# fal-ai-community/video-diffusion-speedrun

Measured on AMD Instinct MI355X. Metric: train-step samples/sec (video latents), higher is better.
Workload: dtype bf16; 1 GPU; C3b DiT-XL/2 bf16, latents [16,16,64,64] pt=2 -> 8192+16 tokens, ctx [512,4096]; per_gpu_batch=12, global_batch=12, parallelism=single, launch=eager, deterministic=False

## Files before the change

### video_diffusion_speedrun_amd/csrc/config.h

```cpp
#pragma once
#include <cstddef>

namespace vdscfg {
enum Knob {
  GEMM_TILE,
  GEMM_NARROW,
  GEMM_GROUP_M,
  GEMM_GROUP_M_TN,
  GEMM_TN_JOINT,
  GEMM_MID_TN,
  GEMM_MID_FACTOR,
  ATTN_MFMA16,
  ATTN_DELTA_FOLD,
  ATTN_TAIL_LAST,
  ATTN_FWD_WIDE,
  ATTN_WIDE_STORES,
  ATTN_QSPLIT,
  CROSS_DKV16,
  ATTN8_DQ_WAVES,
  EW_MIN_ROWS,
  EW_WGS,
  RMSNORM_Q4,
  ROPE_TOK,
  ROPE_TILE,
  ADALN_MFMA,
  COMM_ALLPAIRS,
  DETERMINISTIC,
  N_KNOBS
};
extern double g_val[N_KNOBS];
inline double get(Knob k) { return g_val[k]; }
inline int geti(Knob k) { return (int)g_val[k]; }
const char* rccl_path();
}

namespace vdsdet {
inline bool on() { return vdscfg::g_val[vdscfg::DETERMINISTIC] != 0; }
float* workspace(size_t floats, const char* who);
size_t workspace_bytes();
}
```

### video_diffusion_speedrun_amd/csrc/config.hip

```cpp
#include "config.h"
#include "common.h"
#include "../../include/vds.h"
#include <cmath>
#include <cstdint>
#include <cstdlib>
#include <cstring>

namespace vdscfg {
namespace {
struct Def { const char* name; const char* env; double def; };
const Def kDefs[N_KNOBS] = {
    {"gemm_tile", "VDS_GEMM_TILE", 0},
    {"gemm_narrow", "VDS_GEMM_NARROW", 1},
    {"gemm_group_m", "VDS_GEMM_GROUP_M", 4},
    {"gemm_group_m_tn", "VDS_GEMM_GROUP_M_TN", 0},
    {"gemm_tn_joint", "VDS_GEMM_TN_JOINT", 1},
    {"gemm_mid_tn", "VDS_GEMM_MID_TN", 0.75},
    {"gemm_mid_factor", "VDS_GEMM_MID_FACTOR", 1.3},
    {"attn_mfma16", "VDS_ATTN_MFMA16", 7},
    {"attn_delta_fold", "VDS_ATTN_DELTA_FOLD", 1},
    {"attn_tail_last", "VDS_ATTN_TAIL_LAST", 1},
    {"attn_fwd_wide", "VDS_ATTN_FWD_WIDE", 2},
    {"attn_wide_stores", "VDS_ATTN_WIDE_STORES", 1},
    {"attn_qsplit", "VDS_ATTN_QSPLIT", 0},
    {"cross_dkv16", "VDS_CROSS_DKV16", 1},
    {"attn8_dq_waves", "VDS_ATTN8_DQ_WAVES", 4},
    {"ew_min_rows", "VDS_EW_MIN_ROWS", 8},
    {"ew_wgs", "VDS_EW_WGS", 768},
    {"rmsnorm_q4", "VDS_RMSNORM_Q4", 1},
    {"rope_tok", "VDS_ROPE_TOK", 1},
    {"rope_tile", "VDS_ROPE_TILE", 4},
    {"adaln_mfma", "VDS_ADALN_MFMA", 1},
    {"comm_allpairs", nullptr, 0},
    {"deterministic", nullptr, 0},
};
const char* g_rccl_path = nullptr;
const char* env(const char* name) { return name ? getenv(name) : nullptr; }
struct Init {
  Init() {
    for (int i = 0; i < N_KNOBS; ++i) {
      const char* e = env(kDefs[i].env);
      g_val[i] = (e && *e) ? atof(e) : kDefs[i].def;
    }
    const char* s = env("VDS_COMM_SCHEDULE");
    if (s && strcmp(s, "allpairs") == 0) g_val[COMM_ALLPAIRS] = 1;
    g_rccl_path = env("VDS_RCCL_PATH");
  }
};
}
double g_val[N_KNOBS];
static Init g_init;
const char* rccl_path() { return g_rccl_path; }
}

namespace vdsdet {
static float* g_ws = nullptr;
static size_t g_ws_bytes = 0;
float* workspace(size_t floats, const char* who) {
  if (g_ws && floats * 4 <= g_ws_bytes) return g_ws;
  vdserr::set("%s: deterministic mode needs %zu bytes of workspace, vds_set_deterministic was given %zu", who, floats * 4,
              g_ws_bytes);
  return nullptr;
}
size_t workspace_bytes() { return g_ws ? g_ws_bytes : 0; }
}

extern "C" int vds_set_deterministic(int32_t on, void* workspace, size_t workspace_bytes) {
  const int prev = vdscfg::geti(vdscfg::DETERMINISTIC);
  if (on != 0 && on != 1) return VDS_ERR_ARG;
  if (on && (!workspace || ((uintptr_t)workspace & 15) || workspace_bytes < 4096)) return VDS_ERR_ARG;
  vdscfg::g_val[vdscfg::DETERMINISTIC] = on;
  vdsdet::g_ws = on ? (float*)workspace : nullptr;
  vdsdet::g_ws_bytes = on ? workspace_bytes : 0;
  return prev;
}

extern "C" int vds_knob_set(const char* name, double value) {
  if (!name) return VDS_ERR_ARG;
  for (int i = 0; i < vdscfg::N_KNOBS; ++i)
    if (strcmp(name, vdscfg::kDefs[i].name) == 0) {
      if (i == vdscfg::DETERMINISTIC) return VDS_ERR_ARG;
      vdscfg::g_val[i] = value;
      return VDS_OK;
    }
  return VDS_ERR_ARG;
}

extern "C" double vds_knob_get(const char* name) {
  if (name)
    for (int i = 0; i < vdscfg::N_KNOBS; ++i)
      if (strcmp(name, vdscfg::kDefs[i].name) == 0) return vdscfg::g_val[i];
  return NAN;
}
```

### video_diffusion_speedrun_amd/csrc/gemm.hip

```cpp
#include "common.h"
#include "prof.h"
#include "config.h"
#include "../../include/vds.h"
#include <cmath>
#include <cstdint>
#include <cstring>
#include <mutex>
#include <type_traits>

#ifndef VDS_GEMM_AUX_NT
#define VDS_GEMM_AUX_NT 1
#endif
namespace {

constexpr int BM = 128, BN = 128, BK = 64;
constexpr int TILE_BYTES = 16384;
constexpr int EPI_LD = 68;
constexpr int LDS_BYTES = 4 * 64 * EPI_LD * 4;
constexpr int GROUP_M = 8;

struct GemmP {
  int M, N, K;
  const bf16_t* A; long lda;
  const bf16_t* B; long ldb;
  void* C; long ldc;
  void* C2; long ldc2;
  const bf16_t* bias;
  const bf16_t* aux; long ldaux;
  const float* gate; long ldgate;
  int rows_per_batch;
  int row_base;
  int split_k;
  int atomic;
  long slab_stride;
  unsigned a_bytes, b_bytes;
  int tiles_m, tiles_n;
  int group_m;
  int joint_xcd;
  int narrow;
  const float* sa; const float* sb;
  double prof_k;
  unsigned char* e_q; long e_ldq; unsigned char* e_qt; long e_ldqt;
  const float* e_amax_in; float* e_amax_out; float* e_dq_out; int e_fmt; float* e_colsum;
};

__device__ __forceinline__ int swz_kc(int row, int chunk) { return chunk ^ ((row >> 1) & 7); }
__device__ __forceinline__ int swz_km(int krow) { return (krow & 3) | (((krow >> 3) & 1) << 2); }

template <bool KMAJOR>
__device__ __forceinline__ void stage_tile(srd_t rsrc, char* lds_tile, const unsigned voff[4],
                                           unsigned koff, int wave, int lane, int krem) {
  const unsigned base = lds_addr_of(lds_tile) + wave * 4096;
#pragma unroll
  for (int j = 0; j < 4; ++j) {
    unsigned off = voff[j] + koff;
    if constexpr (!KMAJOR) {
      if (krem < BK) {
        const int row = (wave * 4 + j) * 8 + (lane >> 3);
        if (swz_kc(row, lane & 7) * 8 >= krem) off = 0xfffffff0u;
      }
    }
    lds_dma16(rsrc, base + j * 1024, off);
  }
}

template <bool KMAJOR>
__device__ __forceinline__ void stage_offsets(unsigned voff[4], int wave, int lane, long ld, int origin) {
#pragma unroll
  for (int j = 0; j < 4; ++j) {
    int q = wave * 4 + j;
    if constexpr (!KMAJOR) {
      int row = q * 8 + (lane >> 3);
      int chunk = swz_kc(row, lane & 7);
      voff[j] = (unsigned)(((long)(origin + row) * ld + chunk * 8) * 2);
    } else {
      int krow = q * 4 + (lane >> 4);
      int pc = lane & 15;
      int chunk = (((pc >> 1) ^ swz_km(krow)) << 1) | (pc & 1);
      voff[j] = (unsigned)(((long)krow * ld + origin + chunk * 8) * 2);
    }
  }
}

__device__ __forceinline__ bf16x8 frag_kc(const char* tile, int row0, int ks, int lane) {
  int row = row0 + (lane & 15);
  int chunk = swz_kc(row, ks * 4 + (lane >> 4));
  return *reinterpret_cast<const bf16x8*>(tile + row * 128 + chunk * 16);
}
__device__ __forceinline__ bf16x8 frag_km(const char* tile, int col0, int ks, int lane) {
  int g = lane >> 4, i = lane & 15;
  int krow = ks * 32 + 8 * g + (i >> 2);
  int seg = (col0 >> 4) ^ swz_km(krow);
  const char* p = tile + krow * 256 + seg * 32 + (i & 3) * 8;
  s16x4 lo = __builtin_amdgcn_ds_read_tr16_b64_v4i16((__attribute__((address_space(3))) s16x4*)LDS_PTR(p));
  s16x4 hi = __builtin_amdgcn_ds_read_tr16_b64_v4i16((__attribute__((address_space(3))) s16x4*)LDS_PTR(p + 4 * 256));
  s16x8 r = {lo[0], lo[1], lo[2], lo[3], hi[0], hi[1], hi[2], hi[3]};
  return __builtin_bit_cast(bf16x8, r);
}

typedef __attribute__((ext_vector_type(8))) int i32x8;
__device__ __forceinline__ i32x8 frag_kc8(const char* tile, int row0, int lane) {
  const int row = row0 + (lane & 15);
  const int c0 = swz_kc(row, 2 * (lane >> 4));
  const i32x4 lo = *reinterpret_cast<const i32x4*>(tile + row * 128 + c0 * 16);
  const i32x4 hi = *reinterpret_cast<const i32x4*>(tile + row * 128 + (c0 ^ 1) * 16);
  return i32x8{lo[0], lo[1], lo[2], lo[3], hi[0], hi[1], hi[2], hi[3]};
}

constexpr int LUT_N = 4096, LUT_BYTES = LUT_N * 4, LUT_E0 = 114;
__device__ float g_gelu_lut[2][LUT_N];
typedef __attribute__((ext_vector_type(2))) float f32x2;
typedef __attribute__((ext_vector_type(2))) unsigned short u16x2;

__device__ __forceinline__ f32x2 lut_pair(const char* lut, unsigned w) {
  u16x2 m = __builtin_bit_cast(u16x2, w & 0x7fff7fffu);
  m = __builtin_elementwise_sub_sat(m, u16x2{LUT_E0 << 7, LUT_E0 << 7});
  m = __builtin_elementwise_min(m, u16x2{2047, 2047});
  m = m << u16x2{2, 2};
  const unsigned off = __builtin_bit_cast(unsigned, m) | ((w >> 2) & 0x20002000u);
  f32x2 t;
  t[0] = *reinterpret_cast<const float*>(lut + (off & 0xffffu));
  t[1] = *reinterpret_cast<const float*>(lut + (off >> 16));
  return t;
}
__device__ __forceinline__ f32x2 bf2_to_f2(unsigned w) { return f32x2{bflo(w), bfhi(w)}; }
__device__ __forceinline__ unsigned f2_to_bf2(f32x2 v) { return pack_bf2(v[0], v[1]); }

bool ensure_gelu_lut() {
  static std::mutex mu;
  static bool done[64] = {};
  int dev = 0;
  if (hipGetDevice(&dev) != hipSuccess || dev < 0 || dev >= 64) return false;
  std::lock_guard<std::mutex> lk(mu);
  if (done[dev]) return true;
  static float host[2][LUT_N];
  for (int i = 0; i < LUT_N; ++i) {
    const unsigned bits = (unsigned)(((i & 2047) + (LUT_E0 << 7)) | ((i >> 11) << 15)) << 16;
    float xf;
    memcpy(&xf, &bits, 4);
    const double x = xf;
    const double cdf = 0.5 * erfc(-x * 0.70710678118654752440);
    const double pdf = 0.39894228040143267794 * exp(-0.5 * x * x);
    host[0][i] = (float)cdf;
    host[1][i] = (float)(cdf + x * pdf);
  }
  if (hipMemcpyToSymbol(HIP_SYMBOL(g_gelu_lut), host, sizeof(host)) != hipSuccess) return false;
  done[dev] = true;
  return true;
}

__device__ __forceinline__ unsigned cvt4_fp8(int fmt, float a, float b, float c, float d) {
  int w = 0;
  if (fmt == 0) {
    w = __builtin_amdgcn_cvt_pk_fp8_f32(a, b, w, false);
    w = __builtin_amdgcn_cvt_pk_fp8_f32(c, d, w, true);
  } else {
    w = __builtin_amdgcn_cvt_pk_bf8_f32(a, b, w, false);
    w = __builtin_amdgcn_cvt_pk_bf8_f32(c, d, w, true);
  }
  return (unsigned)w;
}

template <int EPI, int WC = 64, int NIT = 8>
__device__ __forceinline__ void epilogue_prefetch(const GemmP& p, int row0, int col0, int lane, u32x4 (&auxr)[NIT]) {
  if constexpr (EPI == VDS_EPI_GATE_RES || EPI == VDS_EPI_DGELU) {
    const int c8 = lane & 7, rin = lane >> 3;
    const int gcol = col0 + c8 * 8;
    const bool cok = gcol < p.N && (WC == 64 || c8 * 8 < WC);
#pragma unroll
    for (int it = 0; it < NIT; ++it) {
      const long grow = row0 + it * 8 + rin;
#if VDS_GEMM_AUX_NT
      auxr[it] = (grow < p.M && cok) ? __builtin_nontemporal_load(reinterpret_cast<const u32x4*>(p.aux + grow * p.ldaux + gcol))
                                     : u32x4{0u, 0u, 0u, 0u};
#else
      auxr[it] = (grow < p.M && cok) ? *reinterpret_cast<const u32x4*>(p.aux + grow * p.ldaux + gcol)
                                     : u32x4{0u, 0u, 0u, 0u};
#endif
    }
  }
}

template <int EPI, bool EMIT = false, bool LUT = false, int WC = 64, int NIT = 8>
__device__ __forceinline__ void epilogue_64x64(const GemmP& p, float* stg, int row0, int col0, int lane,
                                               float (&cs)[8], u32x2 (&ew)[NIT], const u32x4 (&auxr)[NIT],
                                               const char* lut = nullptr) {
  if constexpr (EPI == VDS_EPI_F32) {
    if (p.atomic) {
      const int acol = col0 + lane;
      if (acol < p.N && lane < WC) {
        float* cbase = reinterpret_cast<float*>(p.C) + (long)row0 * p.ldc + acol;
        const int rmax = min(8 * NIT, p.M - row0);
// ... 599 lines not shown
        for (int j = 0; j < 2; ++j) acc[qa * 4 + i][j] = mma(fa[i][ks], fb0[j][ks], acc[qa * 4 + i][j]);
  };
  auto k_tile = [&](int T, auto PAR) {
    constexpr int par = decltype(PAR)::value;
    const char* buf = ring + par * BUF;
    read_a4(buf + SLOT_A0, fa);
    read_b2(buf + SLOT_B0, fb0);
    issue(T + 1, 3, par ^ 1);
    VDS_WAIT_LGKM0();
    VDS_WAIT_VM(6);
    __builtin_amdgcn_s_barrier();
    __builtin_amdgcn_s_setprio(1);
    quad(0);
    __builtin_amdgcn_s_setprio(0);
    __builtin_amdgcn_s_barrier();
    read_a4(buf + SLOT_A1, fa);
    issue(T + 2, 0, par);
    issue(T + 2, 1, par);
    VDS_WAIT_LGKM0();
    VDS_WAIT_VM(6);
    __builtin_amdgcn_s_barrier();
    __builtin_amdgcn_s_setprio(1);
    quad(1);
    __builtin_amdgcn_s_setprio(0);
    __builtin_amdgcn_s_barrier();
  };
  for (int T = kt_begin; T < kt_end; T += 2) {
    k_tile(T, std::integral_constant<int, 0>{});
    if (T + 1 < kt_end) k_tile(T + 1, std::integral_constant<int, 1>{});
  }
  }
  constexpr int NIT = 8;
  constexpr int NSTEP = 16 / NIT;
  constexpr int RSTEP = 8 * NIT;
  u32x4 auxr2[NSTEP][NIT];
#pragma unroll
  for (int st = 0; st < NSTEP; ++st)
    epilogue_prefetch<EPI, G::WCOLS, NIT>(p, m0 + wr * 128 + st * RSTEP, n0 + wc * G::WCOLS, lane, auxr2[st]);
  if (wr == 0) __builtin_amdgcn_s_barrier();
  const bool aux_all = (EPI == VDS_EPI_GATE_RES || EPI == VDS_EPI_DGELU) && m0 + wr * 128 + 128 <= p.M &&
                       n0 + (wc + 1) * G::WCOLS <= p.N;
  if (aux_all) VDS_WAIT_VM(16);
  else VDS_WAIT_VM(0);
  __builtin_amdgcn_s_barrier();

  constexpr int STG_BASE = 0, STG_WAVE = RSTEP * EPI_LD;
  float* stg = reinterpret_cast<float*>(ring + STG_BASE) + wave * STG_WAVE;
  float dq = 1.0f;
  if constexpr (FMT != 0) dq = (p.sa ? *p.sa : 1.0f) * (p.sb ? *p.sb : 1.0f);
  constexpr bool EMIT = (FMT != 0 && (EPI == VDS_EPI_BIAS_GELU || EPI == VDS_EPI_DGELU)) || (FMT == 0 && EPI == VDS_EPI_DGELU);
  float cs[8];
  u32x2 ew[NSTEP][NIT];
#pragma unroll
  for (int e = 0; e < 8; ++e) cs[e] = 0.f;
  [[maybe_unused]] float e_scale = 1.0f, e_max = 0.f;
  if constexpr (EMIT) {
    const float fmax = p.e_fmt == 0 ? 448.0f : 57344.0f;
    const float ain = ((p.e_q || p.e_qt) && p.e_amax_in) ? *p.e_amax_in : 0.f;
    e_scale = ain > 0.f ? fmax / ain : 1.0f;
    if ((p.e_q || p.e_qt) && p.e_dq_out && m0 == 0 && n0 == 0 && tid == 0) *p.e_dq_out = ain > 0.f ? ain / fmax : 1.0f;
  }
  const char* lut = smem;
#pragma unroll
  for (int qa = 0; qa < NSTEP; ++qa) {
    const u32x4 (&auxr)[NIT] = auxr2[qa];
    const int row0 = m0 + wr * 128 + qa * RSTEP, col0 = n0 + wc * WCOLS;
#pragma unroll
    for (int i = 0; i < RSTEP / 16; ++i)
#pragma unroll
      for (int j = 0; j < NJ; ++j) {
        f32x4 v = acc[qa * (RSTEP / 16) + i][j];
        if constexpr (FMT != 0) v *= dq;
        *reinterpret_cast<f32x4*>(stg + (i * 16 + (lane & 15)) * EPI_LD + j * 16 + 4 * (lane >> 4)) = v;
      }
    VDS_WAIT_LGKM0();
    __builtin_amdgcn_wave_barrier();
    bool full = row0 + RSTEP <= p.M && col0 + WCOLS <= p.N;
    if constexpr (EPI == VDS_EPI_GATE_RES) full = full && ((row0 + p.row_base) % p.rows_per_batch) + RSTEP <= p.rows_per_batch;
    if constexpr (EPI == VDS_EPI_F32) full = false;
    bool done = false;
    if (full) done = epilogue_full_dispatch<EPI, EMIT, WCOLS, NIT>(p, stg, lut, row0, col0, lane, cs, ew[qa], auxr, e_scale, e_max);
    if (!done) epilogue_64x64<EPI, EMIT, USE_LUT, WCOLS, NIT>(p, stg, row0, col0, lane, cs, ew[qa], auxr, lut);
    __builtin_amdgcn_wave_barrier();
  }
  if constexpr (EMIT) {
    if ((p.e_q || p.e_qt) && p.e_amax_out) {
#pragma unroll
      for (int o = 32; o > 0; o >>= 1) e_max = fmaxf(e_max, __shfl_xor(e_max, o));
      unsigned* a = reinterpret_cast<unsigned*>(p.e_amax_out);
      if (lane == 0 && __float_as_uint(e_max) > __atomic_load_n(a, __ATOMIC_RELAXED)) atomicMax(a, __float_as_uint(e_max));
    }
  }
  if constexpr (EMIT) {
    if (p.e_qt) {
      constexpr int TLD = 72;
      unsigned char* bt = reinterpret_cast<unsigned char*>(stg);
      const int c8 = lane & 7, rin = lane >> 3;
#pragma unroll
      for (int qa = 0; qa < NSTEP; ++qa)
#pragma unroll
        for (int it = 0; it < NIT; ++it) *reinterpret_cast<u32x2*>(bt + (qa * RSTEP + it * 8 + rin) * TLD + c8 * 8) = ew[qa][it];
      VDS_WAIT_LGKM0();
      __builtin_amdgcn_wave_barrier();
      const int mq = lane & 31;
      const long m = m0 + wr * 128 + 4 * mq;
#pragma unroll
      for (int it = 0; it < 8; ++it) {
        const int kq = (lane >> 5) + 2 * it;
        unsigned r[4];
#pragma unroll
        for (int i = 0; i < 4; ++i) r[i] = *reinterpret_cast<const unsigned*>(bt + (4 * mq + i) * TLD + 4 * kq);
        const unsigned t0 = __builtin_amdgcn_perm(r[1], r[0], 0x05010400u), t1 = __builtin_amdgcn_perm(r[1], r[0], 0x07030602u);
        const unsigned t2 = __builtin_amdgcn_perm(r[3], r[2], 0x05010400u), t3 = __builtin_amdgcn_perm(r[3], r[2], 0x07030602u);
        const unsigned c[4] = {__builtin_amdgcn_perm(t2, t0, 0x05040100u), __builtin_amdgcn_perm(t2, t0, 0x07060302u),
                               __builtin_amdgcn_perm(t3, t1, 0x05040100u), __builtin_amdgcn_perm(t3, t1, 0x07060302u)};
#pragma unroll
        for (int j = 0; j < 4; ++j) {
          const int col = n0 + wc * WCOLS + 4 * kq + j;
          if (col >= p.N || m >= p.M || 4 * kq + j >= WCOLS) continue;
          unsigned char* dst = p.e_qt + (long)col * p.e_ldqt + m;
          if (m + 4 <= p.M) *reinterpret_cast<unsigned*>(dst) = c[j];
          else
            for (int i = 0; i < (int)(p.M - m); ++i) dst[i] = (unsigned char)(c[j] >> (8 * i));
        }
      }
      VDS_WAIT_LGKM0();
      __builtin_amdgcn_wave_barrier();
    }
    if (p.e_colsum) {
#pragma unroll
      for (int e = 0; e < 8; ++e) {
        cs[e] += __shfl_xor(cs[e], 8);
        cs[e] += __shfl_xor(cs[e], 16);
        cs[e] += __shfl_xor(cs[e], 32);
      }
      if (wr == 1 && lane < 8)
#pragma unroll
        for (int e = 0; e < 8; ++e) stg[lane * 8 + e] = cs[e];
      __syncthreads();
      if (wr == 0 && lane < WCOLS / 8) {
        const float* other = reinterpret_cast<const float*>(ring + STG_BASE) + (wave + 4) * STG_WAVE;
        const int gcol = n0 + wc * WCOLS + lane * 8;
#pragma unroll
        for (int e = 0; e < 8; ++e)
          if (gcol + e < p.N) atomicAdd(p.e_colsum + gcol + e, cs[e] + other[lane * 8 + e]);
      }
    }
  }
}

template <int LAYOUT, int EPI, int FMT = 0>
__global__ __launch_bounds__(512, 2) void gemm_kernel(GemmP p) {
  extern __shared__ __attribute__((aligned(16))) char smem[];
  const int nwg = p.tiles_m * p.tiles_n;
  int pid = blockIdx.x;
  {
    int q = nwg >> 3, r = nwg & 7, xcd = pid & 7, idx = pid >> 3;
    pid = (xcd < r ? xcd * (q + 1) : r * (q + 1) + (xcd - r) * q) + idx;
  }
  const int group = p.group_m * p.tiles_n;
  const int first_m = (pid / group) * p.group_m;
  const int gsz = min(p.tiles_m - first_m, p.group_m);
  const int tile_m = first_m + (pid % group) % gsz;
  const int tile_n = (pid % group) / gsz;
  const int m0 = tile_m * BM, n0 = tile_n * 256;

  const int kt_total = (p.K + BK - 1) / BK;
  int kt_begin = 0, kt_end = kt_total;
  if (p.split_k > 1) {
    int per = (kt_total + p.split_k - 1) / p.split_k;
    kt_begin = blockIdx.y * per;
    kt_end = min(kt_total, kt_begin + per);
    if (kt_begin >= kt_end) return;
  }
  if (p.narrow && tile_n == p.tiles_n - 1) {
    gemm_tile<LAYOUT, EPI, FMT, 128>(p, smem, m0, n0, kt_begin, kt_end);
    return;
  }
  gemm_tile<LAYOUT, EPI, FMT, 256>(p, smem, m0, n0, kt_begin, kt_end);
}

template <int LAYOUT, int EPI, int FMT = 0>
int launch(const GemmP& p, hipStream_t s) {
  constexpr bool USE_LUT = EPI == VDS_EPI_BIAS_GELU || EPI == VDS_EPI_DGELU;
  constexpr int LDS_TOTAL = LDS_BYTES + (USE_LUT ? LUT_BYTES : 0);
  static bool attr_set = false;
  if (!attr_set) {
    (void)hipFuncSetAttribute(reinterpret_cast<const void*>(&gemm_kernel<LAYOUT, EPI, FMT>),
                              hipFuncAttributeMaxDynamicSharedMemorySize, LDS_TOTAL);
    attr_set = true;
  }
  if constexpr (USE_LUT) {
    if (!ensure_gelu_lut()) return VDS_ERR_LAUNCH;
  }
  dim3 grid(p.tiles_m * p.tiles_n, p.split_k > 1 ? p.split_k : 1, 1);
  const double k = FMT != 0 ? p.prof_k : (double)p.K;
  vdsprof::Scope ps(FMT != 0 ? VDS_PROF_GEMM_FP8 : LAYOUT == VDS_NT ? VDS_PROF_GEMM_NT : LAYOUT == VDS_NN ? VDS_PROF_GEMM_NN
                                                                                                       : VDS_PROF_GEMM_TN,
                    s, 2.0 * p.M * p.N * k, (FMT != 0 ? 1.0 : 2.0) * ((double)p.M * k + (double)p.N * k) + 2.0 * (double)p.M * p.N);
  hipLaunchKernelGGL((gemm_kernel<LAYOUT, EPI, FMT>), grid, dim3(512), LDS_TOTAL, s, p);
  return hipGetLastError() == hipSuccess ? VDS_OK : VDS_ERR_LAUNCH;
}

}

namespace mid {
constexpr int BM = 256, BN = 128, BK = 32;
constexpr int A_BYTES = 16384, B_BYTES = 8192, STAGE = A_BYTES + B_BYTES;
constexpr int LDS_BYTES = 3 * STAGE;
static_assert(LDS_BYTES >= 4 * 64 * EPI_LD * 4, "epilogue staging must fit in the stage ring");

__device__ __forceinline__ int swz32(int row) {
  const int h = (row >> 2) & 3;
  return (((h >> 1) ^ h) & 1) << 1 | (h >> 1);
}

template <bool KMAJOR, int ROWS>
__device__ __forceinline__ void offsets(unsigned (&voff)[ROWS / 64], int (&kchunk)[ROWS / 64], int wave, int lane,
                                        long ld, int origin) {
  constexpr int NP = ROWS / 64;
#pragma unroll
  for (int j = 0; j < NP; ++j) {
    const int q = wave * NP + j;
    if constexpr (!KMAJOR) {
      const int row = q * 16 + (lane >> 2);
      const int chunk = (lane & 3) ^ swz32(row);
      kchunk[j] = chunk * 8;
      voff[j] = (unsigned)(((long)(origin + row) * ld + chunk * 8) * 2);
    } else {
      const int t = q >> 3, krow = (q & 7) * 4 + (lane >> 4);
      const int pc = lane & 15;
      const int chunk = (((pc >> 1) ^ swz_km(krow)) << 1) | (pc & 1);
      kchunk[j] = krow;
      voff[j] = (unsigned)(((long)krow * ld + origin + t * 128 + chunk * 8) * 2);
    }
  }
}

template <bool KMAJOR, int NP>
__device__ __forceinline__ void issue(srd_t rsrc, char* slot, const unsigned (&voff)[NP], const int (&kchunk)[NP],
                                      unsigned koff, int krem, int wave) {
  const unsigned base = lds_addr_of(slot) + wave * NP * 1024;
#pragma unroll
  for (int j = 0; j < NP; ++j) {
    unsigned off = voff[j] + koff;
    if (kchunk[j] >= krem) off = 0xfffffff0u;
    lds_dma16(rsrc, base + j * 1024, off);
  }
}

__device__ __forceinline__ bf16x8 frag_kc32(const char* tile, int row0, int lane) {
  const int row = row0 + (lane & 15);
  const int pc = (lane >> 4) ^ swz32(row);
  return *reinterpret_cast<const bf16x8*>(tile + row * 64 + pc * 16);
}

template <int LAYOUT, int EPI>
__global__ __launch_bounds__(256, 2) void gemm_kernel(GemmP p) {
  extern __shared__ __attribute__((aligned(16))) char smem[];
  constexpr bool A_KM = (LAYOUT == VDS_TN);
  constexpr bool B_KM = (LAYOUT != VDS_NT);
  const int tid = threadIdx.x, lane = tid & 63;
  const int wave = __builtin_amdgcn_readfirstlane(tid >> 6);
  const int wm = wave >> 1, wn = wave & 1;

  const int nwg = p.tiles_m * p.tiles_n;
  int pid = blockIdx.x, split = blockIdx.y;
  if (p.split_k > 1 && p.joint_xcd) {
    const int total = nwg * p.split_k;
    int L = blockIdx.y * nwg + blockIdx.x;
    const int q = total >> 3, r = total & 7, xcd = L & 7, idx = L >> 3;
    L = (xcd < r ? xcd * (q + 1) : r * (q + 1) + (xcd - r) * q) + idx;
    split = L / nwg;
    pid = L - split * nwg;
  } else {
    int q = nwg >> 3, r = nwg & 7, xcd = pid & 7, idx = pid >> 3;
    pid = (xcd < r ? xcd * (q + 1) : r * (q + 1) + (xcd - r) * q) + idx;
  }
  const int group = p.group_m * p.tiles_n;
  const int first_m = (pid / group) * p.group_m;
  const int gsz = min(p.tiles_m - first_m, p.group_m);
  const int tile_m = first_m + (pid % group) % gsz;
  const int tile_n = (pid % group) / gsz;
  const int m0 = tile_m * BM, n0 = tile_n * BN;

  const int kt_total = (p.K + BK - 1) / BK;
  int kt_begin = 0, kt_end = kt_total;
  if (p.split_k > 1) {
    int per = (kt_total + p.split_k - 1) / p.split_k;
    kt_begin = split * per;
    kt_end = min(kt_total, kt_begin + per);
    if (kt_begin >= kt_end) return;
  }

  const srd_t ra = make_srd(p.A, p.a_bytes);
  const srd_t rb = make_srd(p.B, p.b_bytes);
  unsigned va[4], vb[2];
  int ca[4], cb[2];
  offsets<A_KM, 256>(va, ca, wave, lane, p.lda, m0);
  offsets<B_KM, 128>(vb, cb, wave, lane, p.ldb, n0);
  const unsigned a_step = A_KM ? (unsigned)(BK * p.lda * 2) : BK * 2;
  const unsigned b_step = B_KM ? (unsigned)(BK * p.ldb * 2) : BK * 2;

  auto stage_in = [&](int T, int slot) {
    const int krem = (T < kt_end) ? p.K - T * BK : 0;
    char* st = smem + slot * STAGE;
    issue<A_KM, 4>(ra, st, va, ca, (unsigned)T * a_step, krem, wave);
    issue<B_KM, 2>(rb, st + A_BYTES, vb, cb, (unsigned)T * b_step, krem, wave);
  };

  f32x4 acc[8][4];
#pragma unroll
  for (int i = 0; i < 8; ++i)
#pragma unroll
    for (int j = 0; j < 4; ++j) acc[i][j] = f32x4{0.f, 0.f, 0.f, 0.f};

  stage_in(kt_begin, 0);
  stage_in(kt_begin + 1, 1);
  VDS_WAIT_VM(6);
  __builtin_amdgcn_s_barrier();

  auto k_step = [&](int T, auto SLOT) {
    constexpr int slot = decltype(SLOT)::value;
    stage_in(T + 2, (slot + 2) % 3);
    const char* ta = smem + slot * STAGE;
    const char* tb = ta + A_BYTES;
    bf16x8 fa[8], fb[4];
#pragma unroll
    for (int i = 0; i < 8; ++i) {
      if constexpr (A_KM) fa[i] = frag_km(ta + wm * B_BYTES, i * 16, 0, lane);
      else fa[i] = frag_kc32(ta, wm * 128 + i * 16, lane);
    }
#pragma unroll
    for (int j = 0; j < 4; ++j) {
      if constexpr (B_KM) fb[j] = frag_km(tb, wn * 64 + j * 16, 0, lane);
      else fb[j] = frag_kc32(tb, wn * 64 + j * 16, lane);
    }
    __builtin_amdgcn_s_setprio(1);
#pragma unroll
    for (int i = 0; i < 8; ++i)
#pragma unroll
      for (int j = 0; j < 4; ++j) acc[i][j] = __builtin_amdgcn_mfma_f32_16x16x32_bf16(fa[i], fb[j], acc[i][j], 0, 0, 0);
    __builtin_amdgcn_s_setprio(0);
    VDS_WAIT_VM(6);
    __builtin_amdgcn_s_barrier();
  };
  for (int T = kt_begin; T < kt_end; T += 3) {
    k_step(T, std::integral_constant<int, 0>{});
    if (T + 1 < kt_end) k_step(T + 1, std::integral_constant<int, 1>{});
    if (T + 2 < kt_end) k_step(T + 2, std::integral_constant<int, 2>{});
  }
  VDS_WAIT_VM(0);
  __builtin_amdgcn_s_barrier();

  float* stg = reinterpret_cast<float*>(smem) + wave * 64 * EPI_LD;
  float cs_unused[8];
  u32x2 ew_unused[8];
#pragma unroll
  for (int qa = 0; qa < 2; ++qa) {
    u32x4 auxr[8];
    epilogue_prefetch<EPI>(p, m0 + wm * 128 + qa * 64, n0 + wn * 64, lane, auxr);
#pragma unroll
    for (int i = 0; i < 4; ++i)
#pragma unroll
      for (int j = 0; j < 4; ++j)
#pragma unroll
        for (int r = 0; r < 4; ++r)
          stg[(i * 16 + 4 * (lane >> 4) + r) * EPI_LD + j * 16 + (lane & 15)] = acc[qa * 4 + i][j][r];
    VDS_WAIT_LGKM0();
    __builtin_amdgcn_wave_barrier();
    epilogue_64x64<EPI>(p, stg, m0 + wm * 128 + qa * 64, n0 + wn * 64, lane, cs_unused, ew_unused, auxr);
    __builtin_amdgcn_wave_barrier();
  }
}

template <int LAYOUT, int EPI>
int launch(const GemmP& p, hipStream_t s) {
  static bool attr_set = false;
  if (!attr_set) {
    (void)hipFuncSetAttribute(reinterpret_cast<const void*>(&gemm_kernel<LAYOUT, EPI>),
                              hipFuncAttributeMaxDynamicSharedMemorySize, LDS_BYTES);
    attr_set = true;
  }
  dim3 grid(p.tiles_m * p.tiles_n, p.split_k > 1 ? p.split_k : 1, 1);
  vdsprof::Scope ps(LAYOUT == VDS_NT ? VDS_PROF_GEMM_NT : LAYOUT == VDS_NN ? VDS_PROF_GEMM_NN : VDS_PROF_GEMM_TN, s,
                    2.0 * p.M * p.N * p.K, 2.0 * ((double)p.M * p.K + (double)p.N * p.K + (double)p.M * p.N));
  hipLaunchKernelGGL((gemm_kernel<LAYOUT, EPI>), grid, dim3(256), LDS_BYTES, s, p);
  return hipGetLastError() == hipSuccess ? VDS_OK : VDS_ERR_LAUNCH;
}
}

thread_local char g_err[256] = "";

template <int LAYOUT, int EPI>
int launch(const GemmP& p, hipStream_t s) {
  static bool attr_set = false;
  if (!attr_set) {
    (void)hipFuncSetAttribute(reinterpret_cast<const void*>(&gemm_kernel<LAYOUT, EPI>),
                              hipFuncAttributeMaxDynamicSharedMemorySize, LDS_BYTES);
    attr_set = true;
  }
  dim3 grid(p.tiles_m * p.tiles_n, p.split_k > 1 ? p.split_k : 1, 1);
  vdsprof::Scope ps(LAYOUT == VDS_NT ? VDS_PROF_GEMM_NT : LAYOUT == VDS_NN ? VDS_PROF_GEMM_NN : VDS_PROF_GEMM_TN, s,
                    2.0 * p.M * p.N * p.K, 2.0 * ((double)p.M * p.K + (double)p.N * p.K + (double)p.M * p.N));
  hipLaunchKernelGGL((gemm_kernel<LAYOUT, EPI>), grid, dim3(256), LDS_BYTES, s, p);
  return hipGetLastError() == hipSuccess ? VDS_OK : VDS_ERR_LAUNCH;
}


__global__ __launch_bounds__(256) void splitk_reduce_kernel(const float* ws, int n_slabs, long slab_stride, float* C, long ldc,
                                                            int M, int N) {
  const long i4 = (long)blockIdx.x * 256 + threadIdx.x;
  const int n4 = N >> 2;
  if (i4 >= (long)M * n4) return;
  const long row = i4 / n4;
  const int col = (int)(i4 % n4) * 4;
  float* c = C + row * ldc + col;
  f32x4 v = *reinterpret_cast<const f32x4*>(c);
  const float* w = ws + row * N + col;
  for (int sidx = 0; sidx < n_slabs; ++sidx) v += *reinterpret_cast<const f32x4*>(w + (long)sidx * slab_stride);
  *reinterpret_cast<f32x4*>(c) = v;
}

inline int force_tile() { return vdscfg::geti(vdscfg::GEMM_TILE); }

inline int narrow_last_column(long N) {
  if (!vdscfg::geti(vdscfg::GEMM_NARROW)) return 0;
  const long rem = N % 256;
  return rem > 0 && rem <= 128;
}

template <typename F>
int launch_split_det(GemmP& p, float* C, long ldc, hipStream_t s, int bk, F launch_fn) {
  const int kt_total = cdiv(p.K, bk);
  int split = p.split_k;
  const size_t slab = (size_t)p.M * p.N * 4;
  while (split > 1 && (size_t)split * slab > vdsdet::workspace_bytes()) --split;
  if (split <= 1) {
    p.split_k = 1;
    return launch_fn(p);
  }
  const int per = cdiv(kt_total, split);
  const int n_eff = cdiv(kt_total, per);
  float* ws = vdsdet::workspace((size_t)split * p.M * p.N, "vds_gemm (split-K)");
  if (!ws) return VDS_ERR_ARG;
  p.split_k = split;
  p.atomic = 0;
  p.joint_xcd = 0;
  p.C = ws;
  p.ldc = p.N;
  p.slab_stride = (long)p.M * p.N;
  const int rc = launch_fn(p);
  if (rc != VDS_OK) return rc;
  const long n4 = (long)p.M * (p.N >> 2);
  hipLaunchKernelGGL(splitk_reduce_kernel, dim3((unsigned)((n4 + 255) / 256)), dim3(256), 0, s, (const float*)ws, n_eff,
                     p.slab_stride, C, ldc, p.M, p.N);
  return hipGetLastError() == hipSuccess ? VDS_OK : VDS_ERR_LAUNCH;
}

}

extern "C" int vds_gemm_force_tile(int32_t tile) {
  const int prev = force_tile();
  if (tile != 0 && tile != 128 && tile != 256 && tile != 2) return VDS_ERR_ARG;
  vdscfg::g_val[vdscfg::GEMM_TILE] = tile;
  return prev;
}

extern "C" int vds_gemm_bf16(const vds_gemm_args* a, vds_stream_t stream) {
  if (!a || !a->A || !a->B || a->M <= 0 || a->N <= 0 || a->K <= 0) return VDS_ERR_ARG;
  if ((a->N & 7) || (a->lda & 7) || (a->ldb & 7)) return VDS_ERR_ARG;
  GemmP p;
  p.M = a->M; p.N = a->N; p.K = a->K;
  p.A = (const bf16_t*)a->A; p.lda = a->lda;
  p.B = (const bf16_t*)a->B; p.ldb = a->ldb;
  p.C = a->C; p.ldc = a->ldc; p.C2 = a->C2; p.ldc2 = a->ldc2;
  p.bias = (const bf16_t*)a->bias;
  p.aux = (const bf16_t*)a->aux; p.ldaux = a->ldaux;
  p.gate = a->gate; p.ldgate = a->ldgate;
  p.rows_per_batch = a->rows_per_batch > 0 ? a->rows_per_batch : a->M;
  p.row_base = 0;
  p.slab_stride = 0;
  const bool auto_split = (a->split_k == 0 || a->split_k == -1) && a->layout == VDS_TN && a->epilogue == VDS_EPI_F32;
  p.split_k = a->split_k > 1 ? a->split_k : (a->split_k < -1 ? -a->split_k : 1);
  p.atomic = (a->split_k > 1 || a->split_k < 0) ? 1 : 0;
  p.sa = p.sb = nullptr;
  p.prof_k = a->K;
  p.e_q = p.e_qt = nullptr; p.e_ldq = p.e_ldqt = 0;
  p.e_amax_in = nullptr; p.e_amax_out = p.e_dq_out = p.e_colsum = nullptr; p.e_fmt = 0;
  p.narrow = 0;
  if (a->colsum && !(a->epilogue == VDS_EPI_DGELU && a->C)) return VDS_ERR_ARG;
  p.tiles_m = cdiv(a->M, BM);
  p.tiles_n = cdiv(a->N, BN);
  size_t abytes, bbytes;
  switch (a->layout) {
    case VDS_NT:
      if (a->K & 7) return VDS_ERR_ARG;
      abytes = ((size_t)(a->M - 1) * a->lda + a->K) * 2;
      bbytes = ((size_t)(a->N - 1) * a->ldb + a->K) * 2;
      break;
    case VDS_NN:
      if (a->K & 7) return VDS_ERR_ARG;
      abytes = ((size_t)(a->M - 1) * a->lda + a->K) * 2;
      bbytes = ((size_t)(a->K - 1) * a->ldb + a->N) * 2;
      break;
    case VDS_TN:
      if (a->M & 7) return VDS_ERR_ARG;
      abytes = ((size_t)(a->K - 1) * a->lda + a->M) * 2;
      bbytes = ((size_t)(a->K - 1) * a->ldb + a->N) * 2;
      break;
    default:
      return VDS_ERR_ARG;
  }
  if (abytes >= (1ull << 32) || bbytes >= (1ull << 32)) return VDS_ERR_UNSUPPORTED;
  p.a_bytes = (unsigned)abytes;
  p.b_bytes = (unsigned)bbytes;
  hipStream_t s = (hipStream_t)stream;
  if (p.atomic && !(a->layout == VDS_TN && a->epilogue == VDS_EPI_F32)) return VDS_ERR_ARG;
  if (!a->C && !((a->epilogue == VDS_EPI_GATE_RES || a->epilogue == VDS_EPI_BIAS_GELU) && a->C2)) return VDS_ERR_ARG;
  const bool det = vdscfg::geti(vdscfg::DETERMINISTIC) != 0;
  const float* fused_colsum = det ? nullptr : a->colsum;
  const int ft = force_tile();
  const int tm = cdiv(a->M, 256), tn = cdiv(a->N, 256);
  const long rounds_big = ((long)tm * tn + 255) / 256;
  const long rounds_small = ((long)p.tiles_m * p.tiles_n + 511) / 512;
  bool use_big = a->layout != VDS_TN && a->K >= 256 && (double)rounds_big * (2.0 / 1.24) < (double)rounds_small;
  if (ft == 128) use_big = false;
  if (ft == 256 && a->layout != VDS_TN) use_big = true;
  p.group_m = vdscfg::geti(vdscfg::GEMM_GROUP_M);
  if (p.group_m < 1) p.group_m = 4;
  p.joint_xcd = 0;
  const int group_m_tn = vdscfg::geti(vdscfg::GEMM_GROUP_M_TN) > 0 ? vdscfg::geti(vdscfg::GEMM_GROUP_M_TN) : 0;
  if (a->layout == VDS_TN) {
    p.group_m = group_m_tn ? group_m_tn : 2;
    p.joint_xcd = vdscfg::geti(vdscfg::GEMM_TN_JOINT);
  }
  auto launch_tn = [&](int bk, auto fn) -> int {
    if (det && p.split_k > 1) return launch_split_det(p, (float*)a->C, a->ldc, s, bk, fn);
    return fn(p);
  };
  if (auto_split) {
    const double mid_tn = vdscfg::get(vdscfg::GEMM_MID_TN);
    const long kt = cdiv(a->K, 64);
    double best = 1e300;
    int best_tile = 128, best_s = 1;
    for (int cand = 0; cand < 2; ++cand) {
      if ((cand == 0 && ft == 2) || (cand == 1 && ft == 128)) continue;
      const long tiles = cand == 0 ? (long)cdiv(a->M, 128) * cdiv(a->N, 128) : (long)cdiv(a->M, 256) * cdiv(a->N, 128);
      const double unit = cand == 0 ? 1.0 : 2.0 * mid_tn, atom = cand == 0 ? 0.034 : 0.068;
      for (int sp = 1; sp <= 32; ++sp) {
        if (sp > 1 && kt / sp < 8) break;
        const long rounds = (tiles * sp + 511) / 512;
        const double cost = (double)rounds * (double)((kt + sp - 1) / sp) * unit + (sp > 1 ? tiles * sp * atom : 0.0);
        if (cost < best - 1e-9) { best = cost; best_tile = cand == 0 ? 128 : 2; best_s = sp; }
      }
    }
    p.split_k = best_s;
    p.atomic = (best_s > 1 || a->split_k == -1) ? 1 : 0;
    if (best_tile == 2) {
      p.tiles_m = cdiv(a->M, 256);
      p.tiles_n = cdiv(a->N, 128);
      if (p.joint_xcd && !group_m_tn) {
        const long chunk = ((long)p.tiles_m * p.tiles_n * p.split_k + 7) / 8;
        long g = (chunk + p.tiles_n / 2) / p.tiles_n;
        p.group_m = (int)(g < 1 ? 1 : (g > p.tiles_m ? p.tiles_m : g));
      }
      return launch_tn(mid::BK, [&](GemmP& q) { return mid::launch<VDS_TN, VDS_EPI_F32>(q, s); });
    }
    return launch_tn(BK, [&](GemmP& q) { return launch<VDS_TN, VDS_EPI_F32>(q, s); });
  }
  {
    const int tmm = cdiv(a->M, 256), tnm = cdiv(a->N, 128);
    const double cost_mid = (double)(((long)tmm * tnm + 511) / 512) * vdscfg::get(vdscfg::GEMM_MID_FACTOR);
    const double cost_big = (double)rounds_big, cost_small = (double)rounds_small * (1.24 / 2.0);
    bool use_mid = a->K >= 128 && cost_mid < (use_big ? cost_big : cost_small) && a->layout != VDS_TN;
    if (ft == 2) use_mid = true;
    if (a->colsum && a->layout != VDS_NN) use_mid = false;
    if (ft == 128 || ft == 256) use_mid = false;
    if (use_mid) {
      p.tiles_m = tmm;
      p.tiles_n = tnm;
      if (a->colsum) {
        const int rc = mid::launch<VDS_NN, VDS_EPI_DGELU>(p, s);
        return rc != VDS_OK ? rc : vds_colsum_bf16(a->C, a->ldc, a->colsum, a->M, a->N, stream);
      }
#define GOM(L, E) if (a->layout == L && a->epilogue == E) return mid::launch<L, E>(p, s);
      GOM(VDS_NT, VDS_EPI_STORE)
      GOM(VDS_NT, VDS_EPI_BIAS_GELU)
      GOM(VDS_NT, VDS_EPI_GATE_RES)
      GOM(VDS_NN, VDS_EPI_STORE)
      GOM(VDS_NN, VDS_EPI_DGELU)
#undef GOM
      if (a->layout == VDS_TN && a->epilogue == VDS_EPI_F32)
        return launch_tn(mid::BK, [&](GemmP& q) { return mid::launch<VDS_TN, VDS_EPI_F32>(q, s); });
    }
  }
  if (use_big) {
    p.tiles_m = tm;
    p.tiles_n = tn;
    p.narrow = narrow_last_column(a->N);
    p.e_colsum = const_cast<float*>(fused_colsum);
    int rc = VDS_ERR_UNSUPPORTED;
#define GOB(L, E) if (a->layout == L && a->epilogue == E) rc = big::launch<L, E>(p, s);
    GOB(VDS_NT, VDS_EPI_STORE)
    GOB(VDS_NT, VDS_EPI_BIAS_GELU)
    GOB(VDS_NT, VDS_EPI_GATE_RES)
    GOB(VDS_NN, VDS_EPI_STORE)
    GOB(VDS_NN, VDS_EPI_DGELU)
#undef GOB
    if (rc == VDS_OK && a->colsum && !fused_colsum) return vds_colsum_bf16(a->C, a->ldc, a->colsum, a->M, a->N, stream);
    return rc;
  }
  p.tiles_m = cdiv(a->M, BM);
  p.tiles_n = cdiv(a->N, BN);
  if (a->colsum) {
    const int rc = launch<VDS_NN, VDS_EPI_DGELU>(p, s);
    return rc != VDS_OK ? rc : vds_colsum_bf16(a->C, a->ldc, a->colsum, a->M, a->N, stream);
  }
#define GO(L, E) if (a->layout == L && a->epilogue == E) return launch<L, E>(p, s);
  GO(VDS_NT, VDS_EPI_STORE)
  GO(VDS_NT, VDS_EPI_BIAS_GELU)
  GO(VDS_NT, VDS_EPI_GATE_RES)
  GO(VDS_NN, VDS_EPI_STORE)
  GO(VDS_NN, VDS_EPI_DGELU)
#undef GO
  if (a->layout == VDS_TN && a->epilogue == VDS_EPI_F32)
    return launch_tn(BK, [&](GemmP& q) { return launch<VDS_TN, VDS_EPI_F32>(q, s); });
  return VDS_ERR_UNSUPPORTED;
}

extern "C" int vds_gemm_fp8(const vds_gemm_args* a, const float* scale_a, const float* scale_b, int32_t a_fmt,
                            int32_t b_fmt, const vds_fp8_out* emit, vds_stream_t stream) {
  if (!a || !a->A || !a->B || a->M <= 0 || a->N <= 0 || a->K <= 0) return VDS_ERR_ARG;
  if ((a->layout != VDS_NT && a->layout != VDS_TN) || b_fmt != 0 || (a_fmt != 0 && a_fmt != 1)) return VDS_ERR_UNSUPPORTED;
  if ((a->N & 7) || (a->K & 15) || (a->lda & 15) || (a->ldb & 15)) return VDS_ERR_ARG;
  const bool tn = a->layout == VDS_TN;
  if (tn && (a->epilogue != VDS_EPI_F32 || a_fmt != 1 || emit || (a->M & 15))) return VDS_ERR_UNSUPPORTED;
  GemmP p;
  p.M = a->M; p.N = a->N; p.K = a->K / 2;
  p.A = (const bf16_t*)a->A; p.lda = a->lda / 2;
  p.B = (const bf16_t*)a->B; p.ldb = a->ldb / 2;
  p.C = a->C; p.ldc = a->ldc; p.C2 = a->C2; p.ldc2 = a->ldc2;
  p.bias = (const bf16_t*)a->bias;
  p.aux = (const bf16_t*)a->aux; p.ldaux = a->ldaux;
  p.gate = a->gate; p.ldgate = a->ldgate;
  p.rows_per_batch = a->rows_per_batch > 0 ? a->rows_per_batch : a->M;
  p.row_base = 0;
  p.slab_stride = 0;
  p.split_k = a->split_k > 1 ? a->split_k : (a->split_k < -1 ? -a->split_k : 1);
  p.atomic = (a->split_k > 1 || a->split_k < 0) ? 1 : 0;
  p.sa = scale_a; p.sb = scale_b;
  p.prof_k = a->K;
  p.tiles_m = cdiv(a->M, 256);
  p.tiles_n = cdiv(a->N, 256);
  const size_t abytes = tn ? (size_t)(a->K - 1) * a->lda + a->M : (size_t)(a->M - 1) * a->lda + a->K;
  const size_t bbytes = tn ? (size_t)(a->K - 1) * a->ldb + a->N : (size_t)(a->N - 1) * a->ldb + a->K;
  if (abytes >= (1ull << 32) || bbytes >= (1ull << 32)) return VDS_ERR_UNSUPPORTED;
  p.a_bytes = (unsigned)abytes;
  p.b_bytes = (unsigned)bbytes;
  p.group_m = 4;
  p.joint_xcd = 0;
  p.narrow = narrow_last_column(a->N);
  p.e_q = p.e_qt = nullptr; p.e_ldq = p.e_ldqt = 0;
  p.e_amax_in = nullptr; p.e_amax_out = p.e_dq_out = p.e_colsum = nullptr; p.e_fmt = 0;
  if (emit) {
    if (a->epilogue != VDS_EPI_BIAS_GELU && a->epilogue != VDS_EPI_DGELU) return VDS_ERR_ARG;
    if ((emit->q && (emit->ldq & 7)) || (emit->qt && (emit->ldqt & 3)) || (emit->fmt != 0 && emit->fmt != 1)) return VDS_ERR_ARG;
    if ((emit->q || emit->qt) && !emit->amax_in) return VDS_ERR_ARG;
    p.e_q = (unsigned char*)emit->q; p.e_ldq = emit->ldq;
    p.e_qt = (unsigned char*)emit->qt; p.e_ldqt = emit->ldqt;
    p.e_amax_in = emit->amax_in; p.e_amax_out = emit->amax_out; p.e_dq_out = emit->dq_out;
    p.e_fmt = emit->fmt; p.e_colsum = emit->colsum;
  }
  if (p.atomic && a->epilogue != VDS_EPI_F32) return VDS_ERR_ARG;
  if (!a->C && a->epilogue != VDS_EPI_GATE_RES && !(emit && a->epilogue == VDS_EPI_DGELU)) return VDS_ERR_ARG;
  hipStream_t s = (hipStream_t)stream;
  if (tn) {
    if (vdscfg::geti(vdscfg::DETERMINISTIC) && p.split_k > 1)
      return launch_split_det(p, (float*)a->C, a->ldc, s, BK, [&](GemmP& q) { return big::launch<VDS_TN, VDS_EPI_F32, 3>(q, s); });
    return big::launch<VDS_TN, VDS_EPI_F32, 3>(p, s);
  }
  if (vdscfg::geti(vdscfg::DETERMINISTIC) && p.e_colsum) return VDS_ERR_UNSUPPORTED;
#define GOF(E, F) if (a->epilogue == E && a_fmt == F - 1) return big::launch<VDS_NT, E, F>(p, s);
  GOF(VDS_EPI_STORE, 1)
  GOF(VDS_EPI_BIAS_GELU, 1)
  GOF(VDS_EPI_GATE_RES, 1)
  GOF(VDS_EPI_STORE, 2)
  GOF(VDS_EPI_DGELU, 2)
  GOF(VDS_EPI_F32, 2)
  GOF(VDS_EPI_F32, 1)
#undef GOF
  return VDS_ERR_UNSUPPORTED;
}
```

Before: 14.75 samples/s.

## Split big-GEMM wave-quantization remainder tiles into half-width workgroups

Adds a remainder planner for the 256x256 big-tile GEMM: when the last partial round of tiles is at most half full, those tiles are split into two 128-wide halves so the tail round spreads across more workgroups. Narrow last columns are launched as a separate trailing range. The big/mid/small selection cost model now uses the fractional round estimate. This targets tail-effect idle CUs, at the cost of more complex tile indexing and a possibly different path choice for some shapes.

```diff
diff --git a/video_diffusion_speedrun_amd/csrc/config.h b/video_diffusion_speedrun_amd/csrc/config.h
--- a/video_diffusion_speedrun_amd/csrc/config.h
+++ b/video_diffusion_speedrun_amd/csrc/config.h
@@ -5,6 +5,7 @@
 enum Knob {
   GEMM_TILE,
   GEMM_NARROW,
+  GEMM_REMAINDER,
   GEMM_GROUP_M,
   GEMM_GROUP_M_TN,
   GEMM_TN_JOINT,
diff --git a/video_diffusion_speedrun_amd/csrc/config.hip b/video_diffusion_speedrun_amd/csrc/config.hip
--- a/video_diffusion_speedrun_amd/csrc/config.hip
+++ b/video_diffusion_speedrun_amd/csrc/config.hip
@@ -12,6 +12,7 @@
 const Def kDefs[N_KNOBS] = {
     {"gemm_tile", "VDS_GEMM_TILE", 0},
     {"gemm_narrow", "VDS_GEMM_NARROW", 1},
+    {"gemm_remainder", "VDS_GEMM_REMAINDER", 1},
     {"gemm_group_m", "VDS_GEMM_GROUP_M", 4},
     {"gemm_group_m_tn", "VDS_GEMM_GROUP_M_TN", 0},
     {"gemm_tn_joint", "VDS_GEMM_TN_JOINT", 1},
diff --git a/video_diffusion_speedrun_amd/csrc/gemm.hip b/video_diffusion_speedrun_amd/csrc/gemm.hip
--- a/video_diffusion_speedrun_amd/csrc/gemm.hip
+++ b/video_diffusion_speedrun_amd/csrc/gemm.hip
@@ -38,6 +38,7 @@
   int group_m;
   int joint_xcd;
   int narrow;
+  int cols_main, wg_main, wg_split;
   const float* sa; const float* sb;
   double prof_k;
   unsigned char* e_q; long e_ldq; unsigned char* e_qt; long e_ldqt;
@@ -943,18 +944,27 @@
 template <int LAYOUT, int EPI, int FMT = 0>
 __global__ __launch_bounds__(512, 2) void gemm_kernel(GemmP p) {
   extern __shared__ __attribute__((aligned(16))) char smem[];
-  const int nwg = p.tiles_m * p.tiles_n;
   int pid = blockIdx.x;
-  {
-    int q = nwg >> 3, r = nwg & 7, xcd = pid & 7, idx = pid >> 3;
-    pid = (xcd < r ? xcd * (q + 1) : r * (q + 1) + (xcd - r) * q) + idx;
-  }
-  const int group = p.group_m * p.tiles_n;
-  const int first_m = (pid / group) * p.group_m;
-  const int gsz = min(p.tiles_m - first_m, p.group_m);
-  const int tile_m = first_m + (pid % group) % gsz;
-  const int tile_n = (pid % group) / gsz;
-  const int m0 = tile_m * BM, n0 = tile_n * 256;
+  int tile_m, tile_n, half = -1;
+  if (pid < p.wg_main + p.wg_split) {
+    if (pid < p.wg_main) {
+      const int nwg = p.wg_main;
+      int q = nwg >> 3, r = nwg & 7, xcd = pid & 7, idx = pid >> 3;
+      pid = (xcd < r ? xcd * (q + 1) : r * (q + 1) + (xcd - r) * q) + idx;
+    } else {
+      half = (pid - p.wg_main) & 1;
+      pid = p.wg_main + ((pid - p.wg_main) >> 1);
+    }
+    const int group = p.group_m * p.cols_main;
+    const int first_m = (pid / group) * p.group_m;
+    const int gsz = min(p.tiles_m - first_m, p.group_m);
+    tile_m = first_m + (pid % group) % gsz;
+    tile_n = (pid % group) / gsz;
+  } else {
+    tile_m = pid - (p.wg_main + p.wg_split);
+    tile_n = p.tiles_n - 1;
+  }
+  const int m0 = tile_m * BM, n0 = tile_n * 256 + (half > 0 ? 128 : 0);
 
   const int kt_total = (p.K + BK - 1) / BK;
   int kt_begin = 0, kt_end = kt_total;
@@ -964,7 +974,7 @@
     kt_end = min(kt_total, kt_begin + per);
     if (kt_begin >= kt_end) return;
   }
-  if (p.narrow && tile_n == p.tiles_n - 1) {
+  if (half >= 0 || (p.narrow && tile_n == p.tiles_n - 1)) {
     gemm_tile<LAYOUT, EPI, FMT, 128>(p, smem, m0, n0, kt_begin, kt_end);
     return;
   }
@@ -984,7 +994,7 @@
   if constexpr (USE_LUT) {
     if (!ensure_gelu_lut()) return VDS_ERR_LAUNCH;
   }
-  dim3 grid(p.tiles_m * p.tiles_n, p.split_k > 1 ? p.split_k : 1, 1);
+  dim3 grid(p.wg_main + p.wg_split + (p.cols_main < p.tiles_n ? p.tiles_m : 0), p.split_k > 1 ? p.split_k : 1, 1);
   const double k = FMT != 0 ? p.prof_k : (double)p.K;
   vdsprof::Scope ps(FMT != 0 ? VDS_PROF_GEMM_FP8 : LAYOUT == VDS_NT ? VDS_PROF_GEMM_NT : LAYOUT == VDS_NN ? VDS_PROF_GEMM_NN
                                                                                                        : VDS_PROF_GEMM_TN,
@@ -1219,6 +1229,30 @@
   if (!vdscfg::geti(vdscfg::GEMM_NARROW)) return 0;
   const long rem = N % 256;
   return rem > 0 && rem <= 128;
+}
+
+struct BigPlan { int cols_main, wg_main, wg_split; double rounds; };
+inline BigPlan plan_big(int tm, int tn, int narrow, bool splittable) {
+  BigPlan b{tn, tm * tn, 0, (double)(((long)tm * tn + 255) / 256)};
+  const int mode = vdscfg::geti(vdscfg::GEMM_REMAINDER);
+  if (!splittable || mode <= 0 || (narrow && mode < 2)) return b;
+  const int cols = tn - (narrow ? 1 : 0);
+  const long T = (long)tm * cols, H = narrow ? tm : 0, F = T / 256, R = T % 256;
+  const bool split = F >= 1 && R > 0 && R <= 128;
+  b.cols_main = cols;
+  b.wg_split = split ? (int)(2 * R) : 0;
+  b.wg_main = (int)(T - (split ? R : 0));
+  double tail;
+  if (split) {
+    tail = 0.5 * (double)((2 * R + H + 255) / 256);
+  } else if (R == 0) {
+    tail = 0.5 * (double)((H + 255) / 256);
+  } else {
+    long h = H - (H < 2 * (256 - R) ? H : 2 * (256 - R));
+    tail = 1.0 + 0.5 * (double)((h + 255) / 256);
+  }
+  b.rounds = (double)F + tail;
+  return b;
 }
 
 template <typename F>
@@ -1280,6 +1314,7 @@
   p.e_q = p.e_qt = nullptr; p.e_ldq = p.e_ldqt = 0;
   p.e_amax_in = nullptr; p.e_amax_out = p.e_dq_out = p.e_colsum = nullptr; p.e_fmt = 0;
   p.narrow = 0;
+  p.cols_main = p.wg_main = p.wg_split = 0;
   if (a->colsum && !(a->epilogue == VDS_EPI_DGELU && a->C)) return VDS_ERR_ARG;
   p.tiles_m = cdiv(a->M, BM);
   p.tiles_n = cdiv(a->N, BN);
@@ -1313,9 +1348,10 @@
   const float* fused_colsum = det ? nullptr : a->colsum;
   const int ft = force_tile();
   const int tm = cdiv(a->M, 256), tn = cdiv(a->N, 256);
-  const long rounds_big = ((long)tm * tn + 255) / 256;
+  const BigPlan bp = plan_big(tm, tn, narrow_last_column(a->N), a->layout != VDS_TN);
+  const double rounds_big = bp.rounds;
   const long rounds_small = ((long)p.tiles_m * p.tiles_n + 511) / 512;
-  bool use_big = a->layout != VDS_TN && a->K >= 256 && (double)rounds_big * (2.0 / 1.24) < (double)rounds_small;
+  bool use_big = a->layout != VDS_TN && a->K >= 256 && rounds_big * (2.0 / 1.24) < (double)rounds_small;
   if (ft == 128) use_big = false;
   if (ft == 256 && a->layout != VDS_TN) use_big = true;
   p.group_m = vdscfg::geti(vdscfg::GEMM_GROUP_M);
@@ -1363,7 +1399,7 @@
   {
     const int tmm = cdiv(a->M, 256), tnm = cdiv(a->N, 128);
     const double cost_mid = (double)(((long)tmm * tnm + 511) / 512) * vdscfg::get(vdscfg::GEMM_MID_FACTOR);
-    const double cost_big = (double)rounds_big, cost_small = (double)rounds_small * (1.24 / 2.0);
+    const double cost_big = rounds_big, cost_small = (double)rounds_small * (1.24 / 2.0);
     bool use_mid = a->K >= 128 && cost_mid < (use_big ? cost_big : cost_small) && a->layout != VDS_TN;
     if (ft == 2) use_mid = true;
     if (a->colsum && a->layout != VDS_NN) use_mid = false;
@@ -1390,6 +1426,7 @@
     p.tiles_m = tm;
     p.tiles_n = tn;
     p.narrow = narrow_last_column(a->N);
+    p.cols_main = bp.cols_main; p.wg_main = bp.wg_main; p.wg_split = bp.wg_split;
     p.e_colsum = const_cast<float*>(fused_colsum);
     int rc = VDS_ERR_UNSUPPORTED;
 #define GOB(L, E) if (a->layout == L && a->epilogue == E) rc = big::launch<L, E>(p, s);
@@ -1452,6 +1489,10 @@
   p.group_m = 4;
   p.joint_xcd = 0;
   p.narrow = narrow_last_column(a->N);
+  {
+    const BigPlan bp = plan_big(p.tiles_m, p.tiles_n, p.narrow, !tn && p.split_k <= 1);
+    p.cols_main = bp.cols_main; p.wg_main = bp.wg_main; p.wg_split = bp.wg_split;
+  }
   p.e_q = p.e_qt = nullptr; p.e_ldq = p.e_ldqt = 0;
   p.e_amax_in = nullptr; p.e_amax_out = p.e_dq_out = p.e_colsum = nullptr; p.e_fmt = 0;
   if (emit) {
```

New measurement: 14.74 samples/s, median of 2. No clear change (-0.0%).
